# Jackz915/PackPPI

Hardware: AMD Instinct MI355X
Metric: sampled residues/sec at 100 diffusion steps (higher is better)
Workload: dtype f32 (dense layers as split-f16: two f16 per operand, three f16 MFMAs per product, fp32 accumulate); 1 GPU; data/T1124_lig.pdb (L=739, 738 true residues), 1 complex per GPU; diffusion_steps=100, proximal=False, residues_per_gpu=738, residues_rank0=738, residues_total=738, mode=ode

## Files before the change

### packppi_amd/csrc/pp_node.hip

```cpp
#include <string.h>

#include "pp_internal.h"
#include <utility>

PP_RANGE_COUNTER
PP_RANGE_READER(pp_node_range_hits)

#define NT 512
#ifndef PP_NODE_GROUPS
#define PP_NODE_GROUPS 1
#endif
#define NG PP_NODE_GROUPS
#define NB (4 * NG)

struct NodeArgs {
    int N;
    const float *rmask;
    const int64_t *rtype;
    const float *bb_sincos;
    const float *sc_mask;
    const uint8_t *m1pi, *m2pi;
    const float *frames;
    const float *embT, *emb_b, *emb_g, *emb_beta;
    float *hV, *S, *msum;
// ... 238 lines not shown
#pragma unroll
            for (int j = 0; j < 4; j++) {
                const float arg = (comp(ts.g[gi], j) * 10000.0f) * fr;
                e[j] = (float)(k < 8 ? sin((double)arg) : cos((double)arg));
            }
            v.g[gi] = f4v{e[0], e[1], e[2], e[3]};
        }
        sm.p[16 + k] = v;
    }
    VN acc = embed_pre35(sm, A, chi, n0);
    VN tacc = vn(0.f);
#pragma unroll
    for (int k = 0; k < 16; k++) tacc = vfma(A.embT[(35 + k) * 128 + f], sm.p[16 + k], tacc);
    VN h = layernorm(sm, rflip, vadd(acc, tacc), A.emb_g[f], A.emb_beta[f]);
    if (ks == 0) {
        store_rows(A.hV, 128, n0, A.N, f, h);
        sm.h[f] = h;
    }
    __syncthreads();
    message_inputs(sm, flip, pre0, A.frames, n0, A.N, A.ptsN, A.PAn, A.PCn);
}

__device__ __forceinline__ float wrap_pi(float x) { return pp_wrap_pi(x); }

typedef _Float16 nh8 __attribute__((ext_vector_type(8)));
typedef float nf4 __attribute__((ext_vector_type(4)));
typedef float nf2 __attribute__((ext_vector_type(2)));
typedef unsigned nu2 __attribute__((ext_vector_type(2)));

#ifndef PP_NU_DEPTH
#define PP_NU_DEPTH 8
#endif
#define PP_NU_DEPTH_MULTI 5
#define NU_S128 144
#define NU_S512 528
#define NU_S32 48
#define NU_INV_LO (1.0f / PP_NU_LO_SCALE)

struct AOpN {
    nh8 hi, lo;
};

struct SmemU {
    _Float16 a_hi[16 * NU_S128], a_lo[16 * NU_S128];
    _Float16 b_hi[16 * NU_S128], b_lo[16 * NU_S128];
    _Float16 c_hi[16 * NU_S512], c_lo[16 * NU_S512];
    float stats[3][8][16][2];
    float pts[16][48];
    _Float16 e_hi[16 * NU_S32], e_lo[16 * NU_S32];
    float fr[16][12];
    float par[NU_P_LAST_TOTAL];
};

struct StepScalars {
    float c_ode, w, c_drift, c_diff;
};
struct TimeEmb {
    float v[16];
};

struct NUpdArgs {
    int N;
    const float *rmask;
    const int64_t *rtype;
    const float *bb_sincos;
    const float *sc_mask;
    const uint8_t *m1pi, *m2pi;
    const float *frames;
    const float *embT;
    const float *wstream, *params;
    const float *hV;
    float *hV_out;
    const float *S, *msum;
    float *ptsN, *PAn, *PCn, *ptsE, *PAe, *PCe, *score;
    unsigned *sat;
};

template <bool LAST>
__device__ constexpr int nu_slot_waves(int s) {
    if (!LAST) return s < 52 ? 8 : 3;
    return s < 36 ? 8 : s < 40 ? 4 : s < 46 ? 1 : s < 55 ? 8 : 2;
}

template <int CL>
__device__ __forceinline__ int nu_phys_slot(int s, int q) {
    if constexpr (CL == 1) return s;
    constexpr int NPS = 16 / CL;
    return s < 36 ? s : s < 36 + NPS ? s + NPS * q : s + (16 - NPS);
}
template <bool LAST, int CL>
__device__ constexpr int nu_logical_waves(int s) {
    if (CL == 1) return nu_slot_waves<LAST>(s);
    return s < 36 + 16 / CL ? 8 : 3;
}
__device__ __forceinline__ void gload_N(const nh8 *__restrict__ wq, int slot, AOpN &a) {
    int off = slot * 128;
    asm volatile("" : "+s"(off));
    const nh8 *p = wq + off;
    a.hi = p[0];
    a.lo = p[64];
}
#define MFMA_N(a, b, c) __builtin_amdgcn_mfma_f32_16x16x32_f16((a), (b), (c), 0, 0, 0)
__device__ __forceinline__ void mm3(const AOpN &a, const nh8 &bh, const nh8 &bl, nf4 &cH, nf4 &cL) {
    cH = MFMA_N(a.hi, bh, cH);
    cL = MFMA_N(a.hi, bl, cL);
    cL = MFMA_N(a.lo, bh, cL);
}
__device__ __forceinline__ nf4 fold(const nf4 &cH, const nf4 &cL) {
    return nf4{fmaf(cL[0], NU_INV_LO, cH[0]), fmaf(cL[1], NU_INV_LO, cH[1]), fmaf(cL[2], NU_INV_LO, cH[2]), fmaf(cL[3], NU_INV_LO, cH[3])};
}
__device__ __forceinline__ void ldB(const _Float16 *hi, const _Float16 *lo, int rowoff, int ks, nh8 &bh, nh8 &bl) {
    bh = *reinterpret_cast<const nh8 *>(hi + rowoff + 32 * ks);
    bl = *reinterpret_cast<const nh8 *>(lo + rowoff + 32 * ks);
}
__device__ __forceinline__ void split2(float x0, float x1, unsigned &hp, unsigned &lp) {
    unsigned a, b, c, d;
    float fa, fb;
    PP_RANGE(x0) PP_RANGE(x1)
    asm("v_cvt_f16_f32 %0, %1" : "=v"(a) : "v"(x0));
    asm("v_cvt_f16_f32 %0, %1" : "=v"(b) : "v"(x1));
    asm("v_cvt_f32_f16 %0, %1" : "=v"(fa) : "v"(a));
    asm("v_cvt_f32_f16 %0, %1" : "=v"(fb) : "v"(b));
    const float d0 = (x0 - fa) * PP_NU_LO_SCALE, d1 = (x1 - fb) * PP_NU_LO_SCALE;
    asm("v_cvt_f16_f32 %0, %1" : "=v"(c) : "v"(d0));
    asm("v_cvt_f16_f32 %0, %1" : "=v"(d) : "v"(d1));
    asm("v_pack_b32_f16 %0, %1, %2" : "=v"(hp) : "v"(a), "v"(b));
    asm("v_pack_b32_f16 %0, %1, %2" : "=v"(lp) : "v"(c), "v"(d));
}
__device__ __forceinline__ void publish4(_Float16 *hi, _Float16 *lo, int off, const nf4 &v) {
    nu2 h, l;
    unsigned h0, l0, h1, l1;
    split2(v[0], v[1], h0, l0);
    split2(v[2], v[3], h1, l1);
    h[0] = h0; h[1] = h1; l[0] = l0; l[1] = l1;
    *reinterpret_cast<nu2 *>(hi + off) = h;
    *reinterpret_cast<nu2 *>(lo + off) = l;
}
__device__ __forceinline__ nf4 relu_sat(const nf4 &v, float &satm) {
    satm = __builtin_fmaxf(__builtin_fmaxf(satm, __builtin_fmaxf(v[0], v[1])), __builtin_fmaxf(v[2], v[3]));
    return nf4{__builtin_amdgcn_fmed3f(v[0], 0.f, 65504.f), __builtin_amdgcn_fmed3f(v[1], 0.f, 65504.f),
               __builtin_amdgcn_fmed3f(v[2], 0.f, 65504.f), __builtin_amdgcn_fmed3f(v[3], 0.f, 65504.f)};
}
__device__ __forceinline__ float xsum_g(float v) {
    v += __shfl_xor(v, 16);
    v += __shfl_xor(v, 32);
    return v;
}
__device__ __forceinline__ nf4 ln128(float (*st)[16][2], int wv, int r, int g, const nf4 &x, const nf4 &gain, const nf4 &beta) {
    const float mw = xsum_g((x[0] + x[1]) + (x[2] + x[3])) * (1.f / 16.f);
    const nf4 d = x - mw;
    const float qw = xsum_g(fmaf(d[0], d[0], d[1] * d[1]) + fmaf(d[2], d[2], d[3] * d[3]));
    if (g == 0) *reinterpret_cast<nf2 *>(st[wv][r]) = nf2{mw, qw};
    __syncthreads();
    float m8[8], msum = 0.f, qsum = 0.f;
#pragma unroll
    for (int v = 0; v < 8; v++) {
        const nf2 t = *reinterpret_cast<const nf2 *>(st[v][r]);
        m8[v] = t[0];
        msum += t[0];
        qsum += t[1];
    }
    const float mean = msum * 0.125f;
    float dm = 0.f;
#pragma unroll
    for (int v = 0; v < 8; v++) dm = fmaf(m8[v] - mean, m8[v] - mean, dm);
    const float var = fmaf(16.f, dm, qsum) * (1.f / 128.f);
    const float rstd = 1.f / sqrtf(var + 1e-5f);
    return (x - mean) * rstd * gain + beta;
}

#define NSTAGE_IF(k, OWN, ACCV, BODY)                                                                                  \
    {                                                                                                                  \
        __builtin_amdgcn_sched_barrier(0);                                                                             \
        if constexpr ((k) + NU_ND < NLOAD) {                                                           \
            constexpr int nw_ = nu_logical_waves<LAST, CL>((k) + NU_ND);                                               \
            if (nw_ == 8 || wv < nw_)                                                                                  \
                gload_N(wq, nu_phys_slot<CL>((k) + NU_ND, clq), AR[((k) + NU_ND) % NU_NRING]);                         \
        }                                                                                                              \
        if (OWN) {                                                                                                     \
            const AOpN &AK = AR[(k) % NU_NRING];                                                                       \
            BODY;                                                                                                      \
            asm volatile("" ::"v"(ACCV[0]));                                                                           \
        }                                                                                                              \
    }
#define NSTAGE(k, ACCV, BODY) NSTAGE_IF(k, true, ACCV, BODY)
#define NTILE4_IF(k0, OWN, cH, cL)                                     \
    NSTAGE_IF((k0) + 0, OWN, cH, mm3(AK, bh[0], bl[0], cH, cL))        \
    NSTAGE_IF((k0) + 1, OWN, cH, mm3(AK, bh[1], bl[1], cH, cL))        \
    NSTAGE_IF((k0) + 2, OWN, cH, mm3(AK, bh[2], bl[2], cH, cL))        \
    NSTAGE_IF((k0) + 3, OWN, cH, mm3(AK, bh[3], bl[3], cH, cL))
#define NTILE4(k0, cH, cL) NTILE4_IF(k0, true, cH, cL)
#define LDB4(HI, LO)                                                                  \
    _Pragma("unroll") for (int ks_ = 0; ks_ < 4; ks_++) ldB(HI, LO, r * NU_S128 + 8 * g, ks_, bh[ks_], bl[ks_]);
#define FOSTAGE(s)                                                                                   \
    NSTAGE(20 + (s), cH, {                                                                           \
        if constexpr ((s) + 1 < 16) ldB(sm.c_hi, sm.c_lo, r * NU_S512 + 8 * g, (s) + 1, fh[((s) + 1) & 1], fl[((s) + 1) & 1]); \
        mm3(AK, fh[(s) & 1], fl[(s) & 1], cH, cL);                                                   \
    })

template <int MODE, int NU_ND, int CL = 1, bool SEEDED = false, bool PINNED = false>
__global__ void __launch_bounds__(512)
k_node_update(NUpdArgs A, float *chi, int step, int sde, const float *noise, int embed_next, StepScalars sp, TimeEmb te_next, PPRng rng,
              PPPin pin) {
    static_assert(CL == 1 || MODE == PP_NU_MID, "only the middle layers have a split form");
    static_assert(!SEEDED || MODE == PP_NU_STEP, "only the reverse step draws noise");
    static_assert(!PINNED || SEEDED, "the pinned step is a seeded one: its fixed rows re-noise with the step's own draws");
    constexpr int NU_NRING = NU_ND + 1;
    constexpr bool LAST = MODE != PP_NU_MID;
    constexpr int NSLOT = LAST ? PP_NU_SLOTS_LAST : PP_NU_SLOTS_MID;
    constexpr int NLOAD = MODE == PP_NU_SCORE ? 46 : CL > 1 ? 36 + 16 / CL + 4 : NSLOT;
    const int clq = CL > 1 ? (int)(blockIdx.x % CL) : 0;
    constexpr int NPAR = LAST ? NU_P_LAST_TOTAL : NU_P_MID_TOTAL;
    extern __shared__ __attribute__((aligned(16))) char smem_raw[];
    SmemU &sm = *reinterpret_cast<SmemU *>(smem_raw);
    const int tid = threadIdx.x, lane = tid & 63, wv = __builtin_amdgcn_readfirstlane(tid >> 6);
    const int r = lane & 15, g = lane >> 4, N = A.N, n0 = (int)(blockIdx.x / CL) * 16;
    const int n = n0 + r, nc = n < N ? n : N - 1;
    const bool live = n < N;
    const int fc = 16 * wv + 4 * g;
    const float *par = sm.par;

    const int srow = tid >> 5, scol = (tid & 31) * 4, sn = n0 + srow < N ? n0 + srow : N - 1;
    const nf4 s4 = *reinterpret_cast<const nf4 *>(A.S + (size_t)sn * 128 + scol);
    const nf4 hv4 = *reinterpret_cast<const nf4 *>(A.hV + (size_t)nc * 128 + fc);
    const float ms = A.msum[nc], rm = A.rmask[nc];
    const nf4 zero4i = {0.f, 0.f, 0.f, 0.f};
    float chi1 = 0.f, scm1 = 0.f, nz1 = 0.f, nz2 = 0.f;
    unsigned char m1raw = 0, m2raw = 0;
    int rt = 0;
    pp_rng_row rrow = {0u, 0u, 0u, 0u};
    unsigned char fixraw = 0;
    float cref = 0.f;
    nf4 spv = zero4i;
    if constexpr (MODE == PP_NU_STEP) {
        spv = nf4{sp.c_ode, sp.w, sp.c_drift, sp.c_diff};
        chi1 = chi[(size_t)nc * 4 + g];
        scm1 = A.sc_mask[(size_t)nc * 4 + g];
        m1raw = A.m1pi[(size_t)nc * 4 + g];
        m2raw = A.m2pi[(size_t)nc * 4 + g];
        if constexpr (PINNED) {
            fixraw = pin.fixed[nc];
            cref = pin.chi_ref[(size_t)nc * 4 + g];
        }
        if constexpr (SEEDED) {
            rrow = rng.tab[nc];
        } else if (sde) {
            const size_t NN = (size_t)N * 4;
            const float *nz = noise + (size_t)step * 2 * NN + (size_t)nc * 4 + g;
            nz1 = nz[0];
            nz2 = nz[NN];
        }
        rt = (int)A.rtype[nc];
    }
    nf4 tailv = {0.f, 0.f, 0.f, 0.f};
    nf4 ev[4] = {tailv, tailv, tailv, tailv};
    const int erow = tid & 15, ern = n0 + erow < N ? n0 + erow : N - 1;
    const bool e_bb = MODE == PP_NU_STEP && tid >= 128 && tid < 144, e_te = MODE == PP_NU_STEP && tid >= 192 && tid < 208;
    {
        const int t48 = tid % 48, row = t48 / 3, rn = n0 + row < N ? n0 + row : N - 1;
        tailv = *reinterpret_cast<const nf4 *>(A.frames + (size_t)rn * 12 + 4 * (t48 - 3 * row));
    }
    nf2 bb0 = {0.f, 0.f}, bb1 = bb0, bb2 = bb0;
    if constexpr (MODE == PP_NU_STEP) {
        const nf2 *bp = reinterpret_cast<const nf2 *>(A.bb_sincos + (size_t)ern * 6);
        bb0 = bp[0]; bb1 = bp[1]; bb2 = bp[2];
    }
    constexpr int NPV = (NPAR / 4 + 511) / 512;
    nf4 pv[NPV];
#pragma unroll
    for (int i = 0; i < NPV; i++) {
        const int q = tid + 512 * i;
        pv[i] = reinterpret_cast<const nf4 *>(A.params)[q < NPAR / 4 ? q : 0];
    }
    const nh8 *wq = reinterpret_cast<const nh8 *>(A.wstream) + (size_t)wv * NSLOT * 128 + lane;
    AOpN AR[NU_NRING];
#pragma unroll
    for (int k = 0; k < NU_ND; k++) gload_N(wq, k, AR[k]);
    __builtin_amdgcn_sched_barrier(0);
    if constexpr (SEEDED) {
        if (wv == 0) {
            const pp_rng_words w = pp_rng_draw(rng.seed_lo, rng.seed_hi, rrow, g, step);
            nz1 = pp_rng_normal(w.o[0], w.o[1]);
            nz2 = pp_rng_normal(w.o[2], w.o[3]);
            if constexpr (PINNED) {
                if (pin.renoise) cref = pp_noised_angle(cref, nz1, nz2, pin.sigma, m1raw != 0, m2raw != 0);
                const bool fx = fixraw != 0;
                chi1 = fx ? cref : chi1;
                m1raw = fx ? 2 : (m1raw != 0 ? 1 : 0);
                m2raw = fx ? 0 : m2raw;
            }
        }
        asm volatile("" : "+v"(nz1), "+v"(nz2));
        if constexpr (PINNED) {
            unsigned mw = m1raw | ((unsigned)m2raw << 8);
            asm volatile("" : "+v"(chi1), "+v"(mw));
            m1raw = (unsigned char)mw;
            m2raw = (unsigned char)(mw >> 8);
        }
    }
// ... 1 lines not shown
    for (int i = 0; i < NPV; i++) {
        const int q = tid + 512 * i;
        if (q < NPAR / 4) reinterpret_cast<nf4 *>(sm.par)[q] = pv[i];
    }
    nf4 oh4 = {0.f, 0.f, 0.f, 0.f};
    if constexpr (MODE == PP_NU_STEP) {
        oh4 = *reinterpret_cast<const nf4 *>(A.embT + (size_t)rt * 128 + fc);
    }
    if (e_te) {
#pragma unroll
        for (int k = 0; k < 16; k++) ev[k >> 2][k & 3] = te_next.v[k];
    } else {
        ev[0] = nf4{bb0[0], bb0[1], bb1[0], bb1[1]};
        ev[1] = nf4{bb2[0], bb2[1], 0.f, 0.f};
    }
    if (tid < 48) reinterpret_cast<nf4 *>(&sm.fr[0][0])[tid] = tailv;
    else if (e_bb) {
        publish4(sm.e_hi, sm.e_lo, erow * NU_S32, ev[0]);
        publish4(sm.e_hi, sm.e_lo, erow * NU_S32 + 4, ev[1]);
    } else if (e_te) {
        publish4(sm.e_hi, sm.e_lo, erow * NU_S32 + 12, nf4{0.f, 0.f, ev[0][0], ev[0][1]});
        publish4(sm.e_hi, sm.e_lo, erow * NU_S32 + 16, nf4{ev[0][2], ev[0][3], ev[1][0], ev[1][1]});
        publish4(sm.e_hi, sm.e_lo, erow * NU_S32 + 20, nf4{ev[1][2], ev[1][3], ev[2][0], ev[2][1]});
        publish4(sm.e_hi, sm.e_lo, erow * NU_S32 + 24, nf4{ev[2][2], ev[2][3], ev[3][0], ev[3][1]});
        publish4(sm.e_hi, sm.e_lo, erow * NU_S32 + 28, nf4{ev[3][2], ev[3][3], 0.f, 0.f});
    }
    publish4(sm.a_hi, sm.a_lo, srow * NU_S128 + scol, s4);
    unsigned satrows = 0xffffu;
    if constexpr (MODE == PP_NU_STEP) {
        const unsigned long long bs = __ballot(scm1 != 0.f);
        const unsigned long long br = __ballot(rm != 0.f && (!PINNED || fixraw == 0));
        satrows = (unsigned)((bs | (bs >> 16) | (bs >> 32) | (bs >> 48)) & br & 0xffffull);
    }
    __syncthreads();

    nh8 bh[4], bl[4];
    nf4 cH, cL;
    float satm = 0.f;
    const nf4 zero4 = zero4i;
    LDB4(sm.a_hi, sm.a_lo)
    cH = zero4; cL = zero4;
    NTILE4(0, cH, cL)
    nf4 x = fold(cH, cL) + *reinterpret_cast<const nf4 *>(par + NU_P_OUTB + fc) * ms + hv4;
    const nf4 h1 = ln128(sm.stats[0], wv, r, g, x, *reinterpret_cast<const nf4 *>(par + NU_P_G0 + fc),
                         *reinterpret_cast<const nf4 *>(par + NU_P_B0 + fc));
    publish4(sm.b_hi, sm.b_lo, r * NU_S128 + fc, h1);
    __syncthreads();
    LDB4(sm.b_hi, sm.b_lo)
#define FFN_IN_TILE(c)                                                                                     \
    cH = zero4; cL = zero4;                                                                                \
    NTILE4(4 + 4 * (c), cH, cL)                                                                            \
    publish4(sm.c_hi, sm.c_lo, r * NU_S512 + 16 * (4 * wv + (c)) + 4 * g,                                  \
             relu_sat(fold(cH, cL) + *reinterpret_cast<const nf4 *>(par + NU_P_FIB + 16 * (4 * wv + (c)) + 4 * g), satm));
    FFN_IN_TILE(0) FFN_IN_TILE(1) FFN_IN_TILE(2) FFN_IN_TILE(3)
    const bool satrow = (satrows >> r) & 1u;
    if (!(satm < 65504.f) && satrow) atomicOr(A.sat, 2u);
    __syncthreads();
    nh8 fh[2], fl[2];
    ldB(sm.c_hi, sm.c_lo, r * NU_S512 + 8 * g, 0, fh[0], fl[0]);
    cH = zero4; cL = zero4;
    FOSTAGE(0) FOSTAGE(1) FOSTAGE(2) FOSTAGE(3) FOSTAGE(4) FOSTAGE(5) FOSTAGE(6) FOSTAGE(7)
    FOSTAGE(8) FOSTAGE(9) FOSTAGE(10) FOSTAGE(11) FOSTAGE(12) FOSTAGE(13) FOSTAGE(14) FOSTAGE(15)
    x = fold(cH, cL) + *reinterpret_cast<const nf4 *>(par + NU_P_FOB + fc) + h1;
    const nf4 h2 = ln128(sm.stats[1], wv, r, g, x, *reinterpret_cast<const nf4 *>(par + NU_P_G1 + fc),
                         *reinterpret_cast<const nf4 *>(par + NU_P_B1 + fc)) * rm;
    if (live && clq == 0 && (MODE != PP_NU_STEP || !embed_next)) *reinterpret_cast<nf4 *>(A.hV_out + (size_t)n * 128 + fc) = h2;
    publish4(sm.a_hi, sm.a_lo, r * NU_S128 + fc, h2);
    __syncthreads();
    LDB4(sm.a_hi, sm.a_lo)

    if constexpr (!LAST) {
        constexpr int NPJ = 4 / CL;
#define NU_PROJ(i)                                                                                                     \
        if constexpr ((i) < NPJ) {                                                                                     \
            cH = zero4; cL = zero4;                                                                                    \
            NTILE4(36 + 4 * (i), cH, cL)                                                                               \
            const int pj = NPJ * clq + (i);                                                                            \
            float *dst = pj == 0 ? A.PAe : pj == 1 ? A.PCe : pj == 2 ? A.PAn : A.PCn;                                  \
            nf4 v = fold(cH, cL);                                                                                      \
            if (pj == 0) v = v + *reinterpret_cast<const nf4 *>(par + NU_P_PAE_B + fc);                                \
            else if (pj == 2) v = v + *reinterpret_cast<const nf4 *>(par + NU_P_PAN_B + fc);                           \
            if (live) *reinterpret_cast<nf4 *>(dst + (size_t)n * 128 + fc) = v;                                        \
        }
        NU_PROJ(0) NU_PROJ(1) NU_PROJ(2) NU_PROJ(3)
#undef NU_PROJ
        if (CL > 1 && clq != 0) return;
        cH = zero4; cL = zero4;
        NTILE4_IF(36 + 4 * NPJ, wv < 3, cH, cL)
        if (wv < 3) {
            const nf4 p = fold(cH, cL) + *reinterpret_cast<const nf4 *>(par + NU_P_PTS_B + fc);
            *reinterpret_cast<nf4 *>(&sm.pts[r][fc]) = p;
            if (live) {
                if (fc < 24) *reinterpret_cast<nf4 *>(A.ptsE + (size_t)n * 48 + fc) = p;
                else *reinterpret_cast<nf4 *>(A.ptsN + (size_t)n * 48 + fc - 24) = p;
            }
        }
        __syncthreads();
        if (tid < 256) {
            const int mm = tid >> 7, q = (tid >> 4) & 7, i = tid & 15, ni = n0 + i;
            if (ni < N) {
                float *pts = mm == 0 ? A.ptsE : A.ptsN;
                const float *fr = sm.fr[i];
                const float px = sm.pts[i][24 * mm + 3 * q], py = sm.pts[i][24 * mm + 3 * q + 1], pz = sm.pts[i][24 * mm + 3 * q + 2];
#pragma unroll
                for (int rr = 0; rr < 3; rr++)
                    pts[(size_t)ni * 48 + 24 + 3 * q + rr] = (fr[3 * rr] * px + fr[3 * rr + 1] * py + fr[3 * rr + 2] * pz) + fr[9 + rr];
            }
        }
        return;
    } else {
        cH = zero4; cL = zero4;
        NTILE4_IF(36, wv < 4, cH, cL)
        if (wv < 4) {
            publish4(sm.c_hi, sm.c_lo, r * NU_S512 + fc, relu_sat(fold(cH, cL) + *reinterpret_cast<const nf4 *>(par + NU_P_DB0 + fc), satm));
        }
        __syncthreads();
        const bool w0 = wv == 0;
        {
            nh8 dh[2], dl[2];
            if (w0) {
                ldB(sm.c_hi, sm.c_lo, r * NU_S512 + 8 * g, 0, dh[0], dl[0]);
                ldB(sm.c_hi, sm.c_lo, r * NU_S512 + 8 * g, 1, dh[1], dl[1]);
            }
            nf4 eH = zero4, eL = zero4;
            cH = zero4; cL = zero4;
            NSTAGE_IF(40, w0, cH, mm3(AK, dh[0], dl[0], cH, cL))
            NSTAGE_IF(41, w0, cH, mm3(AK, dh[1], dl[1], cH, cL))
            NSTAGE_IF(42, w0, eH, mm3(AK, dh[0], dl[0], eH, eL))
            NSTAGE_IF(43, w0, eH, mm3(AK, dh[1], dl[1], eH, eL))
            if (w0) {
                publish4(sm.c_hi, sm.c_lo, r * NU_S512 + 64 + 4 * g, relu_sat(fold(cH, cL) + *reinterpret_cast<const nf4 *>(par + NU_P_DB1 + 4 * g), satm));
                publish4(sm.c_hi, sm.c_lo, r * NU_S512 + 80 + 4 * g, relu_sat(fold(eH, eL) + *reinterpret_cast<const nf4 *>(par + NU_P_DB1 + 16 + 4 * g), satm));
                asm volatile("s_waitcnt lgkmcnt(0)" ::: "memory");
                ldB(sm.c_hi, sm.c_lo, r * NU_S512 + 8 * g, 2, dh[0], dl[0]);
            }
            cH = zero4; cL = zero4;
            NSTAGE_IF(44, w0, cH, mm3(AK, dh[0], dl[0], cH, cL))
            if (w0) {
                publish4(sm.c_hi, sm.c_lo, r * NU_S512 + 96 + 4 * g, relu_sat(fold(cH, cL) + *reinterpret_cast<const nf4 *>(par + NU_P_DB2 + 4 * g), satm));
                asm volatile("s_waitcnt lgkmcnt(0)" ::: "memory");
                ldB(sm.c_hi, sm.c_lo, r * NU_S512 + 8 * g, 3, dh[0], dl[0]);
            }
            cH = zero4; cL = zero4;
            NSTAGE_IF(45, w0, cH, mm3(AK, dh[0], dl[0], cH, cL))
        }
        if (w0) {
            if (!(satm < 65504.f) && satrow) atomicOr(A.sat, 2u);
            const nf4 sc = fold(cH, cL) + *reinterpret_cast<const nf4 *>(par + NU_P_DB3);
            if (g == 0 && live) *reinterpret_cast<nf4 *>(A.score + (size_t)n * 4) = sc;
            if constexpr (MODE == PP_NU_STEP) {
                const float s0 = __shfl(sc[0], r), s1 = __shfl(sc[1], r), s2 = __shfl(sc[2], r), s3 = __shfl(sc[3], r);
                const float sg = g == 0 ? s0 : g == 1 ? s1 : g == 2 ? s2 : s3;
                const float sp_c_ode = spv[0], sp_w = spv[1], sp_c_drift = spv[2], sp_c_diff = spv[3];
                const float sw = sg * sp_w;
#define NU_M1ON (PINNED ? m1raw == 1 : m1raw != 0)
                float yk = chi1;
                if (!sde) {
                    if (NU_M1ON || m2raw != 0) yk = chi1 + sp_c_ode * sw;
                } else {
                    if (NU_M1ON) yk = chi1 + (sp_c_drift * sw + sp_c_diff * nz1);
                    if (m2raw != 0) yk = yk + (sp_c_drift * sw + sp_c_diff * nz2);
                }
#undef NU_M1ON
                float y = wrap_pi(yk) * scm1;
                if constexpr (PINNED) {
                    if (m1raw == 2) y = chi1;
                }
                if (live) chi[(size_t)n * 4 + g] = y;
                if constexpr (PINNED) {
                    if (pin.traj != nullptr && live) pin.traj[(size_t)n * 4 + g] = y;
                }
                if (embed_next) {
                    unsigned hp, lp;
                    split2(sinf(y) * scm1, cosf(y) * scm1, hp, lp);
                    *reinterpret_cast<unsigned *>(sm.e_hi + r * NU_S32 + 6 + 2 * g) = hp;
                    *reinterpret_cast<unsigned *>(sm.e_lo + r * NU_S32 + 6 + 2 * g) = lp;
                }
            }
        }
        if constexpr (MODE != PP_NU_STEP) return;
        if (!embed_next) return;
        __syncthreads();
        nh8 eh, el;
        eh = *reinterpret_cast<const nh8 *>(sm.e_hi + r * NU_S32 + 8 * g);
        el = *reinterpret_cast<const nh8 *>(sm.e_lo + r * NU_S32 + 8 * g);
        cH = zero4; cL = zero4;
        NSTAGE(46, cH, mm3(AK, eh, el, cH, cL))
        const nf4 e0 = fold(cH, cL) + (*reinterpret_cast<const nf4 *>(par + NU_P_EMB_B + fc) + oh4);
        const nf4 h0 = ln128(sm.stats[2], wv, r, g, e0, *reinterpret_cast<const nf4 *>(par + NU_P_EMB_G + fc),
                             *reinterpret_cast<const nf4 *>(par + NU_P_EMB_BETA + fc));
        if (live) *reinterpret_cast<nf4 *>(A.hV_out + (size_t)n * 128 + fc) = h0;
        publish4(sm.b_hi, sm.b_lo, r * NU_S128 + fc, h0);
        __syncthreads();
        LDB4(sm.b_hi, sm.b_lo)
        cH = zero4; cL = zero4;
        NTILE4(47, cH, cL)
        if (live) *reinterpret_cast<nf4 *>(A.PAn + (size_t)n * 128 + fc) = fold(cH, cL) + *reinterpret_cast<const nf4 *>(par + NU_P_PAN0_B + fc);
        cH = zero4; cL = zero4;
        NTILE4(51, cH, cL)
        if (live) *reinterpret_cast<nf4 *>(A.PCn + (size_t)n * 128 + fc) = fold(cH, cL);
        if (wv < 2) {
            cH = zero4; cL = zero4;
            NTILE4(55, cH, cL)
            if (fc < 24) {
                const nf4 p = fold(cH, cL) + *reinterpret_cast<const nf4 *>(par + NU_P_PTS0_B + fc);
                *reinterpret_cast<nf4 *>(&sm.pts[r][fc]) = p;
                if (live) *reinterpret_cast<nf4 *>(A.ptsN + (size_t)n * 48 + fc) = p;
            }
        }
        __syncthreads();
        if (tid < 128) {
            const int q = tid >> 4, i = tid & 15, ni = n0 + i;
            if (ni < N) {
                const float *fr = sm.fr[i];
                const float px = sm.pts[i][3 * q], py = sm.pts[i][3 * q + 1], pz = sm.pts[i][3 * q + 2];
#pragma unroll
                for (int rr = 0; rr < 3; rr++)
                    A.ptsN[(size_t)ni * 48 + 24 + 3 * q + rr] = (fr[3 * rr] * px + fr[3 * rr + 1] * py + fr[3 * rr + 2] * pz) + fr[9 + rr];
            }
        }
    }
}

#ifndef PP_EDGE_F16
struct UpdW {
    const float *outT, *out_b;
    const float *g0, *b0, *g1, *b1;
    const float *ffn_inT, *ffn_in_b, *ffn_outT, *ffn_out_b;
    PreW pre_edge, pre_next;
    const float *d0_inT, *d0_in_b, *d0_outT, *d0_out_b, *d2_inT, *d2_in_b, *d2_outT, *d2_out_b;
};

struct WSet {
    float v[32];
};
template <int KL, int DST0 = 0>
__device__ __forceinline__ void wload(WSet &w, const float *__restrict__ WT, int ldo, int col, int k0, float after) {
    int off = (k0 >> 2) * ldo + col;
    asm volatile("" : "+v"(off) : "v"(after));
    const float4 *w4 = reinterpret_cast<const float4 *>(WT);
#pragma unroll
    for (int i = 0; i < KL / 4; i++) {
        const float4 q = w4[off + i * ldo];
        w.v[DST0 + 4 * i] = q.x; w.v[DST0 + 4 * i + 1] = q.y; w.v[DST0 + 4 * i + 2] = q.z; w.v[DST0 + 4 * i + 3] = q.w;
    }
}
template <int KL, int SRC0 = 0>
__device__ __forceinline__ VN wdot(const WSet &w, const VN *act, VN acc) {
#pragma unroll
    for (int i = 0; i < KL; i++) {
        acc = vfma(w.v[SRC0 + i], act[i], acc);
        if ((i & 7) == 7) VN_FOR asm volatile("" : "+v"(acc.g[gi].x), "+v"(acc.g[gi].y), "+v"(acc.g[gi].z), "+v"(acc.g[gi].w));
    }
    return acc;
}

#define ACC_PIN(a) VN_FOR asm volatile("" : "+v"(a.g[gi].x), "+v"(a.g[gi].y), "+v"(a.g[gi].z), "+v"(a.g[gi].w))
__device__ __forceinline__ void wdot4(const WSet &w0, const WSet &w1, const WSet &w2, const WSet &w3, const VN *act,
                                      VN &a0, VN &a1, VN &a2, VN &a3) {
#pragma unroll
    for (int i = 0; i < 32; i++) {
        const VN x = act[i];
        a0 = vfma(w0.v[i], x, a0);
        a1 = vfma(w1.v[i], x, a1);
        a2 = vfma(w2.v[i], x, a2);
        a3 = vfma(w3.v[i], x, a3);
        if ((i & 3) == 3) { ACC_PIN(a0); ACC_PIN(a1); ACC_PIN(a2); ACC_PIN(a3); }
    }
}

__device__ __forceinline__ void message_inputs_pre(Smem &sm, int &flip, const WSet &wA, const WSet &wC, const WSet &wP,
                                                   float in_b, float pts_b, const float *frames, int n0, int N, float *pts,
                                                   float *PA, float *PC) {
    const int f = threadIdx.x & 127, ks = threadIdx.x >> 7;
    const VN *h = sm.h + ks * 32;
    VN *buf = sm.part[flip];
    flip ^= 1;
    buf[ks * 384 + f] = wdot<32>(wA, h, vn(0.f));
    buf[ks * 384 + 128 + f] = wdot<32>(wC, h, vn(0.f));
    if (f < 24) buf[ks * 384 + 256 + f] = wdot<32>(wP, h, vn(0.f));
    __syncthreads();
    if (ks == 0) {
        VN a = vadd(vadd(buf[f], buf[384 + f]), vadd(buf[768 + f], buf[1152 + f]));
        store_rows(PA, 128, n0, N, f, vadd(a, vn(in_b)));
    } else if (ks == 1) {
        VN c = vadd(vadd(buf[128 + f], buf[512 + f]), vadd(buf[896 + f], buf[1280 + f]));
        store_rows(PC, 128, n0, N, f, c);
    } else if (ks == 2 && f < 24) {
        VN p = vadd(vadd(buf[256 + f], buf[640 + f]), vadd(buf[1024 + f], buf[1408 + f]));
        p = vadd(p, vn(pts_b));
        sm.p[f] = p;
        store_rows(pts, 48, n0, N, f, p);
    }
    __syncthreads();
    if (threadIdx.x < 8 * NB) {
        int q = threadIdx.x / NB, i = threadIdx.x % NB;
        int n = n0 + i;
        if (n < N) {
            const float *fr = frames + (size_t)n * 12;
            float x = vcomp(sm.p[3 * q], i), y = vcomp(sm.p[3 * q + 1], i), z = vcomp(sm.p[3 * q + 2], i);
            for (int r = 0; r < 3; r++)
                pts[(size_t)n * 48 + 24 + 3 * q + r] = (fr[3 * r] * x + fr[3 * r + 1] * y + fr[3 * r + 2] * z) + fr[9 + r];
        }
// ... 228 lines not shown
            sm.p[t] = vmul(sv, mk);
        }
        VN acc = vn(wb.v[30]);
        VN_FOR {
            const int b = n0 + 4 * gi;
            const int t0 = b + 0 < N ? (int)A.rtype[b + 0] : 0, t1 = b + 1 < N ? (int)A.rtype[b + 1] : 0;
            const int t2 = b + 2 < N ? (int)A.rtype[b + 2] : 0, t3 = b + 3 < N ? (int)A.rtype[b + 3] : 0;
            acc.g[gi].x += A.embT[t0 * 128 + f]; acc.g[gi].y += A.embT[t1 * 128 + f];
            acc.g[gi].z += A.embT[t2 * 128 + f]; acc.g[gi].w += A.embT[t3 * 128 + f];
        }
        __syncthreads();
#pragma unroll
        for (int k = 0; k < 14; k++) acc = vfma(wb.v[k], sm.p[k], acc);
        const float *te = te_next.v;
        float tacc = 0.f;
#pragma unroll
        for (int k = 0; k < 16; k++) tacc = fmaf(wb.v[14 + k], te[k], tacc);
        VN e = vadd(acc, vn(tacc));
        VN h = layernorm(sm, rflip, e, A.emb_g[f], A.emb_beta[f]);
        if (ks == 0) {
            store_rows(A.hV, 128, n0, N, f, h);
            sm.h[f] = h;
        }
        __syncthreads();
    }
    message_inputs_pre(sm, flip, wa, wd, we, in_b_1, pts_b_1, A.frames, n0, N, A.ptsN, A.PAn, A.PCn);
}

#endif

static NodeArgs make_args(pp_ctx *c) {
    const pp_plan *p = c->plan;
    NodeArgs A;
    A.N = c->N;
    A.rmask = c->b.residue_mask;
    A.rtype = c->b.residue_type;
    A.bb_sincos = c->b.BB_D_sincos;
    A.sc_mask = c->b.SC_D_mask;
    A.m1pi = c->b.chi_1pi_periodic_mask;
    A.m2pi = c->b.chi_2pi_periodic_mask;
    A.frames = c->frames;
    A.embT = p->node_emb_T;
    A.emb_b = p->w + p->off.node_emb_b;
    A.emb_g = p->w + p->off.norm_nodes_g;
    A.emb_beta = p->w + p->off.norm_nodes_b;
    A.hV = c->hV; A.S = c->S; A.msum = c->msum;
    A.ptsN = c->ptsN; A.PAn = c->PAn; A.PCn = c->PCn;
    A.ptsE = c->ptsE; A.PAe = c->PAe; A.PCe = c->PCe;
    A.score = c->score;
    return A;
}
static PreW make_pre(const pp_plan *p, int layer, bool edge) {
    const LayerOff &o = p->off.layer[layer];
    const LayerT &t = p->lt[layer];
    PreW w;
    w.ptsT = edge ? t.pts_edge_wT : t.pts_node_wT;
    w.pts_b = p->w + (edge ? o.pts_edge_b : o.pts_node_b);
    w.AT = edge ? t.em_A_T : t.nm_A_T;
    w.CT = edge ? t.em_C_T : t.nm_C_T;
    w.in_b = p->w + (edge ? o.em_in_b : o.nm_in_b);
    return w;
}

template <typename F>
struct NuInstance {
    int mode, depth, split;
    bool seeded, pinned;
    F fn;
};
typedef void (*nu_kernel_t)(NUpdArgs, float *, int, int, const float *, int, StepScalars, TimeEmb, PPRng, PPPin);
static const NuInstance<nu_kernel_t> nu_table[] = {
    {PP_NU_STEP, PP_NU_DEPTH_MULTI, 1, false, false, k_node_update<PP_NU_STEP, PP_NU_DEPTH_MULTI>},
    {PP_NU_SCORE, PP_NU_DEPTH_MULTI, 1, false, false, k_node_update<PP_NU_SCORE, PP_NU_DEPTH_MULTI>},
    {PP_NU_MID, PP_NU_DEPTH_MULTI, 1, false, false, k_node_update<PP_NU_MID, PP_NU_DEPTH_MULTI>},
    {PP_NU_STEP, PP_NU_DEPTH, 1, false, false, k_node_update<PP_NU_STEP, PP_NU_DEPTH>},
    {PP_NU_SCORE, PP_NU_DEPTH, 1, false, false, k_node_update<PP_NU_SCORE, PP_NU_DEPTH>},
    {PP_NU_MID, PP_NU_DEPTH, 1, false, false, k_node_update<PP_NU_MID, PP_NU_DEPTH>},
    {PP_NU_STEP, PP_NU_DEPTH_MULTI, 1, true, false, k_node_update<PP_NU_STEP, PP_NU_DEPTH_MULTI, 1, true>},
    {PP_NU_STEP, PP_NU_DEPTH, 1, true, false, k_node_update<PP_NU_STEP, PP_NU_DEPTH, 1, true>},
    {PP_NU_STEP, PP_NU_DEPTH_MULTI, 1, true, true, k_node_update<PP_NU_STEP, PP_NU_DEPTH_MULTI, 1, true, true>},
    {PP_NU_STEP, PP_NU_DEPTH, 1, true, true, k_node_update<PP_NU_STEP, PP_NU_DEPTH, 1, true, true>},
    {PP_NU_MID, PP_NU_DEPTH, 4, false, false, k_node_update<PP_NU_MID, PP_NU_DEPTH, 4>},
    {PP_NU_MID, PP_NU_DEPTH, 2, false, false, k_node_update<PP_NU_MID, PP_NU_DEPTH, 2>},
};
#ifndef PP_EDGE_F16
typedef void (*nv_kernel_t)(NodeArgs, UpdW, float *, int, int, const float *, int, PreW, StepScalars, TimeEmb, PPRng, PPPin);
static const NuInstance<nv_kernel_t> nv_table[] = {
    {PP_NU_MID, 0, 1, false, false, k_node_update_valu<PP_NU_MID>},
    {PP_NU_STEP, 0, 1, false, false, k_node_update_valu<PP_NU_STEP>},
    {PP_NU_SCORE, 0, 1, false, false, k_node_update_valu<PP_NU_SCORE>},
    {PP_NU_STEP, 0, 1, true, false, k_node_update_valu<PP_NU_STEP, true>},
    {PP_NU_STEP, 0, 1, true, true, k_node_update_valu<PP_NU_STEP, true, true>},
};
#endif
template <typename F, size_t n>
static F nu_find(const NuInstance<F> (&tab)[n], int mode, int depth, int split, bool seeded, bool pinned) {
    for (const NuInstance<F> &k : tab)
        if (k.mode == mode && k.depth == depth && k.split == split && k.seeded == seeded && k.pinned == pinned) return k.fn;
    return nullptr;
}
static int g_nu_cus = 0;
static pp_status node_attrs() {
    static bool done = false;
    if (!done) {
        PP_HIP_CHECK(hipFuncSetAttribute(reinterpret_cast<const void *>(k_node_embed),
                                         hipFuncAttributeMaxDynamicSharedMemorySize, (int)sizeof(Smem)));
        PP_HIP_CHECK(hipFuncSetAttribute(reinterpret_cast<const void *>(k_node_embed_rows),
                                         hipFuncAttributeMaxDynamicSharedMemorySize, (int)sizeof(Smem)));
        for (const auto &k : nu_table)
            PP_HIP_CHECK(hipFuncSetAttribute(reinterpret_cast<const void *>(k.fn), hipFuncAttributeMaxDynamicSharedMemorySize, (int)sizeof(SmemU)));
#ifndef PP_EDGE_F16
        for (const auto &k : nv_table)
            PP_HIP_CHECK(hipFuncSetAttribute(reinterpret_cast<const void *>(k.fn), hipFuncAttributeMaxDynamicSharedMemorySize, (int)sizeof(Smem)));
#endif
        int dev = 0;
        hipDeviceProp_t prop;
        if (hipGetDevice(&dev) == hipSuccess && hipGetDeviceProperties(&prop, dev) == hipSuccess) g_nu_cus = prop.multiProcessorCount;
        if (g_nu_cus <= 0) g_nu_cus = 256;
        done = true;
    }
    return PP_OK;
}

pp_status pp_launch_node_embed(pp_ctx *c, const float *chi, const StepParams &sp, hipStream_t s) {
    pp_status st = node_attrs();
    if (st != PP_OK) return st;
    NodeArgs A = make_args(c);
    PreW pre0 = make_pre(c->plan, 0, false);
    PP_LAUNCH(c, k_node_embed, dim3((c->N + NB - 1) / NB), dim3(NT), sizeof(Smem), s, A, pre0, chi, sp);
    PP_HIP_CHECK(hipGetLastError());
    return PP_OK;
}

pp_status pp_launch_node_embed_rows(pp_ctx *c, const float *chi, const float *t_rows, hipStream_t s) {
    pp_status st = node_attrs();
    if (st != PP_OK) return st;
    NodeArgs A = make_args(c);
    PreW pre0 = make_pre(c->plan, 0, false);
    TimeFreq fq;
    const float nemb = (float)(-(log(10000.0) / 7.0));
    for (int i = 0; i < 8; i++) fq.v[i] = expf((float)i * nemb);
    hipLaunchKernelGGL(k_node_embed_rows, dim3((c->N + NB - 1) / NB), dim3(NT), sizeof(Smem), s, A, pre0, chi, t_rows, fq);
    PP_HIP_CHECK(hipGetLastError());
    return PP_OK;
}

pp_status pp_launch_node_update(pp_ctx *c, int layer, int last_mode, const NodeEval &ev, hipStream_t s) {
    float *const chi = ev.chi;
    const int step = ev.step;
    const float *const noise = ev.noise;
    const StepParams *cur = last_mode != PP_NU_MID ? ev.cur : nullptr, *next = last_mode == PP_NU_STEP ? ev.next : nullptr;
    const bool pinned = ev.pin != nullptr && last_mode == PP_NU_STEP;
    if (pinned && (ev.rng == nullptr || ev.rng->tab == nullptr || ev.pin->fixed == nullptr || ev.pin->chi_ref == nullptr)) {
        pp_set_error("pp_launch_node_update: the pinned reverse step needs the rng table, fixed and chi_ref");
        return PP_ERR_INVALID;
    }
    const bool seeded = ev.rng != nullptr && ev.rng->tab != nullptr && last_mode == PP_NU_STEP && (ev.mode == PP_MODE_SDE || pinned);
    const PPRng rg = seeded ? *ev.rng : PPRng{nullptr, 0u, 0u};
    const PPPin pn = pinned ? *ev.pin : PPPin{nullptr, nullptr, nullptr, 0.f, 0};
    pp_status st0 = node_attrs();
    if (st0 != PP_OK) return st0;
    if ((last_mode == PP_NU_MID) != (layer < 2)) {
        pp_set_error("pp_launch_node_update: layers 0 and 1 are middle layers, layer 2 is the last one");
        return PP_ERR_INVALID;
    }
    const pp_plan *p = c->plan;
    const LayerT &t = p->lt[layer];
    NUpdArgs A;
    A.N = c->N;
    A.rmask = c->b.residue_mask;
    A.rtype = c->b.residue_type;
    A.bb_sincos = c->b.BB_D_sincos;
    A.sc_mask = c->b.SC_D_mask;
    A.m1pi = c->b.chi_1pi_periodic_mask;
    A.m2pi = c->b.chi_2pi_periodic_mask;
    A.frames = c->frames;
    A.embT = p->node_emb_T;
    A.wstream = t.nu_stream;
    A.params = t.nu_params;
    A.hV = c->hV; A.hV_out = c->hV; A.S = c->S; A.msum = c->msum;
    A.ptsN = c->ptsN; A.PAn = c->PAn; A.PCn = c->PCn;
    A.ptsE = c->ptsE; A.PAe = c->PAe; A.PCe = c->PCe;
    A.score = c->score;
    A.sat = c->sat;
    const int embed_next = next != nullptr ? 1 : 0;
    const dim3 grid((c->N + 15) / 16), block(512);
    const int sde = ev.mode == PP_MODE_SDE ? 1 : 0;
    StepScalars sp = {0.f, 0.f, 0.f, 0.f};
    TimeEmb te = {};
    if (cur) sp = {cur->c_ode, cur->w, cur->c_drift, cur->c_diff};
    if (next) memcpy(te.v, next->temb, sizeof(te.v));
#ifndef PP_EDGE_F16
    {
        static const bool f16_node = PP_GETENV("PP_NODE_F16") != nullptr;
        if (!f16_node) {
            const LayerOff &o = p->off.layer[layer];
            NodeArgs NA = make_args(c);
            UpdW W;
            W.outT = t.nm_out_T; W.out_b = p->w + o.nm_out_b;
            W.g0 = p->w + o.norm_g[0]; W.b0 = p->w + o.norm_b[0];
            W.g1 = p->w + o.norm_g[1]; W.b1 = p->w + o.norm_b[1];
            W.ffn_inT = t.nd_in_T; W.ffn_in_b = p->w + o.nd_in_b;
            W.ffn_outT = t.nd_out_T; W.ffn_out_b = p->w + o.nd_out_b;
            W.pre_edge = make_pre(p, layer, true);
            W.pre_next = make_pre(p, layer < 2 ? layer + 1 : 0, false);
            W.d0_inT = p->d0_in_T; W.d0_in_b = p->w + p->off.d0_in_b;
            W.d0_outT = p->d0_out_T; W.d0_out_b = p->w + p->off.d0_out_b;
            W.d2_inT = p->d2_in_T; W.d2_in_b = p->w + p->off.d2_in_b;
            W.d2_outT = p->d2_out_T; W.d2_out_b = p->w + p->off.d2_out_b;
            const PreW pre0 = make_pre(p, 0, false);
            const dim3 vgrid((c->N + NB - 1) / NB), vblock(NT);
            const nv_kernel_t kv = nu_find(nv_table, last_mode, 0, 1, seeded, pinned);
            if (!kv) FAIL(PP_ERR_UNSUPPORTED, "pp_launch_node_update: no such instance of k_node_update_valu");
            PP_LAUNCH(c, kv, vgrid, vblock, sizeof(Smem), s, NA, W, chi, step, sde, noise, embed_next, pre0, sp, te, rg, pn);
            PP_HIP_CHECK(hipGetLastError());
            return PP_OK;
        }
    }
#endif
    const bool multi = (int)grid.x > g_nu_cus;
    static const char *split_env = PP_GETENV("PP_NU_SPLIT");
    static const int split_max = split_env ? atoi(split_env) : 4;
    const int tiles = (int)grid.x;
    const int cl = last_mode != PP_NU_MID ? 1 : (split_max >= 4 && 4 * tiles <= g_nu_cus) ? 4 : (split_max >= 2 && 2 * tiles <= g_nu_cus) ? 2 : 1;
    if (cl > 1) {
        A.hV_out = c->hV_alt;
        std::swap(c->hV, c->hV_alt);
    }
    const nu_kernel_t kern = nu_find(nu_table, last_mode, cl > 1 || !multi ? PP_NU_DEPTH : PP_NU_DEPTH_MULTI, cl, seeded, pinned);
    if (!kern) FAIL(PP_ERR_UNSUPPORTED, "pp_launch_node_update: no such instance of k_node_update");
    PP_LAUNCH(c, kern, dim3(tiles * cl), block, sizeof(SmemU), s, A, chi, step, sde, noise, embed_next, sp, te, rg, pn);
    PP_HIP_CHECK(hipGetLastError());
    return PP_OK;
}

__global__ void k_rng_table(pp_rng_row *__restrict__ tab, int N, const int32_t *__restrict__ seg_off, int n_seg,
                            const uint64_t *__restrict__ keys) {
    const int n = blockIdx.x * blockDim.x + threadIdx.x;
    if (n >= N) return;
    const int ord = pp_seg_of_row(seg_off, n_seg, n);
    const int start = pp_seg_start(seg_off, ord, n);
    const uint64_t key = keys ? keys[ord] : (uint64_t)ord;
    pp_rng_row t;
    t.row = (uint32_t)(n - start);
    t.pad = 0u;
    t.ckey_lo = (uint32_t)key;
    t.ckey_hi = (uint32_t)(key >> 32);
    tab[n] = t;
}

__global__ void k_noise_seeded(const pp_rng_row *__restrict__ tab, int N, uint32_t seed_lo, uint32_t seed_hi, int step,
                               float *__restrict__ noise, uint32_t *__restrict__ words) {
    const int i = blockIdx.x * blockDim.x + threadIdx.x;
    if (i >= N * 4) return;
    const pp_rng_words w = pp_rng_draw(seed_lo, seed_hi, tab[i >> 2], i & 3, step);
    noise[i] = pp_rng_normal(w.o[0], w.o[1]);
    noise[(size_t)N * 4 + i] = pp_rng_normal(w.o[2], w.o[3]);
    if (words) *reinterpret_cast<uint4 *>(words + (size_t)i * 4) = make_uint4(w.o[0], w.o[1], w.o[2], w.o[3]);
}

__global__ void k_add_noise_seeded(const pp_rng_row *__restrict__ tab, int N, const float *__restrict__ chi0, float sigma,
                                   const uint8_t *__restrict__ m1pi, const uint8_t *__restrict__ m2pi, uint32_t seed_lo,
                                   uint32_t seed_hi, float *__restrict__ chi) {
    const int i = blockIdx.x * blockDim.x + threadIdx.x;
    if (i >= N * 4) return;
    const bool m1 = m1pi[i] != 0, m2 = m2pi[i] != 0;
    float x = chi0[i];
    if (m1 || m2) {
        const pp_rng_words w = pp_rng_draw(seed_lo, seed_hi, tab[i >> 2], i & 3, -1);
        x = pp_noised_angle(x, pp_rng_normal(w.o[0], w.o[1]), pp_rng_normal(w.o[2], w.o[3]), sigma, m1, m2);
    }
    chi[i] = x;
}

pp_status pp_launch_rng_table(pp_ctx *c, bool keys_set, hipStream_t s) {
    hipLaunchKernelGGL(k_rng_table, dim3((c->N + 255) / 256), dim3(256), 0, s, c->rng_tab, c->N, c->seg_off,
                       c->B, keys_set ? c->rng_keys : nullptr);
    PP_HIP_CHECK(hipGetLastError());
    c->rng_tab_set = true;
    return PP_OK;
}

pp_status pp_launch_noise_seeded(pp_ctx *c, uint64_t seed, int step, float *noise, uint32_t *words, hipStream_t s) {
    hipLaunchKernelGGL(k_noise_seeded, dim3((c->N * 4 + 255) / 256), dim3(256), 0, s, c->rng_tab, c->N, (uint32_t)seed,
                       (uint32_t)(seed >> 32), step, noise, words);
    PP_HIP_CHECK(hipGetLastError());
    return PP_OK;
}

pp_status pp_launch_add_noise_seeded(pp_ctx *c, const float *chi0, float sigma, uint64_t seed, float *chi, hipStream_t s) {
    hipLaunchKernelGGL(k_add_noise_seeded, dim3((c->N * 4 + 255) / 256), dim3(256), 0, s, c->rng_tab, c->N, chi0, sigma,
                       c->b.chi_1pi_periodic_mask, c->b.chi_2pi_periodic_mask, (uint32_t)seed, (uint32_t)(seed >> 32), chi);
    PP_HIP_CHECK(hipGetLastError());
    return PP_OK;
}

struct AffArgs {
    const int64_t *rtype;
    const float *sc_sincos;
    const int64_t *mut_mask;
    const float *hV_pret;
    const float *mut_bias, *seq_emb, *f0T, *f0_b, *f2T, *f2_b;
};

__global__ void __launch_bounds__(NT)
k_affinity_embed(NodeArgs A, PreW pre0, AffArgs F) {
    extern __shared__ __attribute__((aligned(16))) char smem_raw[];
// ... 71 lines not shown
```

Before: 64200 residues/s.

## Split middle-layer node update into four projection workgroups plus a points workgroup

Adds a five-workgroup split per 16-row tile for the middle node-update layers. Four workgroups each compute one projection, and a dedicated fifth workgroup computes the points projection. Before, workgroup 0 of the four-way split did both its projection and the points tile. The split is chosen by default when five workgroups per tile fit in the CU count. This shortens the critical-path workgroup, at the cost of a fifth workgroup repeating the shared 36-slot prefix loads and compute.

```diff
diff --git a/packppi_amd/csrc/pp_node.hip b/packppi_amd/csrc/pp_node.hip
--- a/packppi_amd/csrc/pp_node.hip
+++ b/packppi_amd/csrc/pp_node.hip
@@ -344,14 +344,24 @@
     return s < 36 ? 8 : s < 40 ? 4 : s < 46 ? 1 : s < 55 ? 8 : 2;
 }
 
-template <int CL>
+#define NU_ROLE_ALL 0
+#define NU_ROLE_PROJ 1
+#define NU_ROLE_PTS 2
+template <int CL, int ROLE>
 __device__ __forceinline__ int nu_phys_slot(int s, int q) {
-    if constexpr (CL == 1) return s;
-    constexpr int NPS = 16 / CL;
-    return s < 36 ? s : s < 36 + NPS ? s + NPS * q : s + (16 - NPS);
-}
-template <bool LAST, int CL>
+    if constexpr (ROLE == NU_ROLE_ALL) {
+        if constexpr (CL == 1) return s;
+        constexpr int NPS = 16 / CL;
+        return s < 36 ? s : s < 36 + NPS ? s + NPS * q : s + (16 - NPS);
+    } else if constexpr (ROLE == NU_ROLE_PROJ) {
+        return s < 36 ? s : s + 4 * q;
+    } else {
+        return s < 36 ? s : s + 16;
+    }
+}
+template <bool LAST, int CL, int ROLE>
 __device__ constexpr int nu_logical_waves(int s) {
+    if (ROLE != NU_ROLE_ALL) return s < 36 || ROLE == NU_ROLE_PROJ ? 8 : 3;
     if (CL == 1) return nu_slot_waves<LAST>(s);
     return s < 36 + 16 / CL ? 8 : 3;
 }
@@ -435,9 +445,9 @@
     {                                                                                                                  \
         __builtin_amdgcn_sched_barrier(0);                                                                             \
         if constexpr ((k) + NU_ND < NLOAD) {                                                           \
-            constexpr int nw_ = nu_logical_waves<LAST, CL>((k) + NU_ND);                                               \
+            constexpr int nw_ = nu_logical_waves<LAST, CL, ROLE>((k) + NU_ND);                                         \
             if (nw_ == 8 || wv < nw_)                                                                                  \
-                gload_N(wq, nu_phys_slot<CL>((k) + NU_ND, clq), AR[((k) + NU_ND) % NU_NRING]);                         \
+                gload_N(wq, nu_phys_slot<CL, ROLE>((k) + NU_ND, clq), AR[((k) + NU_ND) % NU_NRING]);                   \
         }                                                                                                              \
         if (OWN) {                                                                                                     \
             const AOpN &AK = AR[(k) % NU_NRING];                                                                       \
@@ -460,23 +470,24 @@
         mm3(AK, fh[(s) & 1], fl[(s) & 1], cH, cL);                                                   \
     })
 
-template <int MODE, int NU_ND, int CL = 1, bool SEEDED = false, bool PINNED = false>
-__global__ void __launch_bounds__(512)
-k_node_update(NUpdArgs A, float *chi, int step, int sde, const float *noise, int embed_next, StepScalars sp, TimeEmb te_next, PPRng rng,
-              PPPin pin) {
+template <int MODE, int NU_ND, int CL, bool SEEDED, bool PINNED, int ROLE>
+__device__ __forceinline__ void nu_body(NUpdArgs A, float *chi, int step, int sde, const float *noise, int embed_next, StepScalars sp,
+                                        TimeEmb te_next, PPRng rng, PPPin pin) {
     static_assert(CL == 1 || MODE == PP_NU_MID, "only the middle layers have a split form");
+    static_assert(ROLE == NU_ROLE_ALL || CL == 4, "roles: 4 projection workgroups + the points workgroup");
     static_assert(!SEEDED || MODE == PP_NU_STEP, "only the reverse step draws noise");
     static_assert(!PINNED || SEEDED, "the pinned step is a seeded one: its fixed rows re-noise with the step's own draws");
     constexpr int NU_NRING = NU_ND + 1;
     constexpr bool LAST = MODE != PP_NU_MID;
     constexpr int NSLOT = LAST ? PP_NU_SLOTS_LAST : PP_NU_SLOTS_MID;
-    constexpr int NLOAD = MODE == PP_NU_SCORE ? 46 : CL > 1 ? 36 + 16 / CL + 4 : NSLOT;
-    const int clq = CL > 1 ? (int)(blockIdx.x % CL) : 0;
+    constexpr int NWG = ROLE == NU_ROLE_ALL ? CL : CL + 1;
+    constexpr int NLOAD = MODE == PP_NU_SCORE ? 46 : ROLE != NU_ROLE_ALL ? 36 + 4 : CL > 1 ? 36 + 16 / CL + 4 : NSLOT;
+    const int clq = ROLE == NU_ROLE_PTS ? CL : NWG > 1 ? (int)(blockIdx.x % NWG) : 0;
     constexpr int NPAR = LAST ? NU_P_LAST_TOTAL : NU_P_MID_TOTAL;
     extern __shared__ __attribute__((aligned(16))) char smem_raw[];
     SmemU &sm = *reinterpret_cast<SmemU *>(smem_raw);
     const int tid = threadIdx.x, lane = tid & 63, wv = __builtin_amdgcn_readfirstlane(tid >> 6);
-    const int r = lane & 15, g = lane >> 4, N = A.N, n0 = (int)(blockIdx.x / CL) * 16;
+    const int r = lane & 15, g = lane >> 4, N = A.N, n0 = (int)(blockIdx.x / NWG) * 16;
     const int n = n0 + r, nc = n < N ? n : N - 1;
     const bool live = n < N;
     const int fc = 16 * wv + 4 * g;
@@ -644,11 +655,15 @@
             else if (pj == 2) v = v + *reinterpret_cast<const nf4 *>(par + NU_P_PAN_B + fc);                           \
             if (live) *reinterpret_cast<nf4 *>(dst + (size_t)n * 128 + fc) = v;                                        \
         }
-        NU_PROJ(0) NU_PROJ(1) NU_PROJ(2) NU_PROJ(3)
+        if constexpr (ROLE != NU_ROLE_PTS) {
+            NU_PROJ(0) NU_PROJ(1) NU_PROJ(2) NU_PROJ(3)
+        }
 #undef NU_PROJ
-        if (CL > 1 && clq != 0) return;
+        if constexpr (ROLE == NU_ROLE_PROJ) return;
+        if (ROLE == NU_ROLE_ALL && CL > 1 && clq != 0) return;
+        constexpr int PT0 = ROLE == NU_ROLE_PTS ? 36 : 36 + 4 * NPJ;
         cH = zero4; cL = zero4;
-        NTILE4_IF(36 + 4 * NPJ, wv < 3, cH, cL)
+        NTILE4_IF(PT0, wv < 3, cH, cL)
         if (wv < 3) {
             const nf4 p = fold(cH, cL) + *reinterpret_cast<const nf4 *>(par + NU_P_PTS_B + fc);
             *reinterpret_cast<nf4 *>(&sm.pts[r][fc]) = p;
@@ -781,6 +796,20 @@
                     A.ptsN[(size_t)ni * 48 + 24 + 3 * q + rr] = (fr[3 * rr] * px + fr[3 * rr + 1] * py + fr[3 * rr + 2] * pz) + fr[9 + rr];
             }
         }
+    }
+}
+
+template <int MODE, int NU_ND, int CL = 1, bool SEEDED = false, bool PINNED = false>
+__global__ void __launch_bounds__(512)
+k_node_update(NUpdArgs A, float *chi, int step, int sde, const float *noise, int embed_next, StepScalars sp, TimeEmb te_next, PPRng rng,
+              PPPin pin) {
+    if constexpr (CL == 5) {
+        if ((int)(blockIdx.x % 5) == 4)
+            nu_body<MODE, NU_ND, 4, SEEDED, PINNED, NU_ROLE_PTS>(A, chi, step, sde, noise, embed_next, sp, te_next, rng, pin);
+        else
+            nu_body<MODE, NU_ND, 4, SEEDED, PINNED, NU_ROLE_PROJ>(A, chi, step, sde, noise, embed_next, sp, te_next, rng, pin);
+    } else {
+        nu_body<MODE, NU_ND, CL, SEEDED, PINNED, NU_ROLE_ALL>(A, chi, step, sde, noise, embed_next, sp, te_next, rng, pin);
     }
 }
 
@@ -1175,6 +1204,7 @@
     {PP_NU_STEP, PP_NU_DEPTH, 1, true, true, k_node_update<PP_NU_STEP, PP_NU_DEPTH, 1, true, true>},
     {PP_NU_MID, PP_NU_DEPTH, 4, false, false, k_node_update<PP_NU_MID, PP_NU_DEPTH, 4>},
     {PP_NU_MID, PP_NU_DEPTH, 2, false, false, k_node_update<PP_NU_MID, PP_NU_DEPTH, 2>},
+    {PP_NU_MID, PP_NU_DEPTH, 5, false, false, k_node_update<PP_NU_MID, PP_NU_DEPTH, 5>},
 };
 #ifndef PP_EDGE_F16
 typedef void (*nv_kernel_t)(NodeArgs, UpdW, float *, int, int, const float *, int, PreW, StepScalars, TimeEmb, PPRng, PPPin);
@@ -1313,9 +1343,10 @@
 #endif
     const bool multi = (int)grid.x > g_nu_cus;
     static const char *split_env = PP_GETENV("PP_NU_SPLIT");
-    static const int split_max = split_env ? atoi(split_env) : 4;
+    static const int split_max = split_env ? atoi(split_env) : 5;
     const int tiles = (int)grid.x;
-    const int cl = last_mode != PP_NU_MID ? 1 : (split_max >= 4 && 4 * tiles <= g_nu_cus) ? 4 : (split_max >= 2 && 2 * tiles <= g_nu_cus) ? 2 : 1;
+    const int cl = last_mode != PP_NU_MID ? 1 : (split_max >= 5 && 5 * tiles <= g_nu_cus) ? 5 : (split_max >= 4 && 4 * tiles <= g_nu_cus) ? 4
+                   : (split_max >= 2 && 2 * tiles <= g_nu_cus) ? 2 : 1;
     if (cl > 1) {
         A.hV_out = c->hV_alt;
         std::swap(c->hV, c->hV_alt);
```

Result: no change. 64550 residues/s, median of 6 (+0.6%).
